# angelocatalani/neural-network-compression

Hardware: AMD Instinct MI355X
Metric: weights/sec through prune+k-means (K=256) (higher is better)
Workload: dtype f32

## Files before the change

### neural_network_compression_amd/csrc/nnc_layer.hip

```cpp
#include <hip/hip_runtime.h>

#include <algorithm>
#include <cmath>
#include <cstdint>
#include <cstring>
#include <string>
#include <vector>

#include "nnc.h"

int nnc_set_error_(int code, const char *msg);
int nnc_publish_bytes_(const void *src_dev, void *dst_host_mapped, int nbytes, void *host_ticket, uint64_t ticket, void *stream);
int nnc_wait_ticket_(void *host_ticket, uint64_t ticket, void *stream);
int nnc_sort_pruned_bounded_flagged_(const float *x, int64_t n, int64_t n_neg, int64_t n_zero, float vmin, float vmax, float thr,
                                     float *sorted_out, void *ws, size_t ws_bytes, int32_t *flag_dev, void *stream);
extern "C" int nnc_host_linspace_f32(float start, float stop, int32_t num, float *out)
{
    if (num < 0 || (num > 0 && !out)) return nnc_set_error_(NNC_EINVAL, "nnc_host_linspace_f32: bad argument");
    if (num == 0) return NNC_OK;
    const int div = num - 1;
    const volatile float delta = stop - start;
    if (div > 0) {
        const volatile float step = delta / (float)div;
        for (int i = 0; i < num; i++) {
            volatile float y = (float)i;
            if (step == 0.0f) { y = y / (float)div; y = y * delta; }
            else y = y * step;
            y = y + start;
            out[i] = y;
        }
        out[num - 1] = stop;
    } else {
        volatile float y = 0.0f;
        y = y * delta;
        y = y + start;
        out[0] = y;
    }
    return NNC_OK;
}

static void linspace_f64(double start, double stop, int num, double *out)
{
    const int div = num - 1;
    const volatile double delta = stop - start;
    if (div > 0) {
        const volatile double step = delta / (double)div;
        for (int i = 0; i < num; i++) {
            volatile double y = (double)i;
            if (step == 0.0) { y = y / (double)div; y = y * delta; }
            else y = y * step;
            y = y + start;
            out[i] = y;
        }
        out[num - 1] = stop;
    } else if (num == 1) {
        volatile double y = 0.0;
        y = y * delta;
        out[0] = y + start;
    }
}

extern "C" int nnc_host_cdf(const float *steps32, const int64_t *counts31, float *xnew300, double *cdf300)
{
    if (!steps32 || !counts31 || !xnew300 || !cdf300) return nnc_set_error_(NNC_EINVAL, "nnc_host_cdf: null pointer");
    const float *x = steps32;
    int64_t tot = 0;
// ... 108 lines not shown
    L.total = o + 256;
    return L;
}

extern "C" size_t nnc_compress_layer_workspace_bytes(int64_t n, int32_t k)
{
    if (n < 1 || k < 1 || k > NNC_KMAX - 8) return 0;
    return layer_layout(n, k).total;
}

extern "C" size_t nnc_compress_layer_host_bytes(void) { return 24576; }

#define LCHK(call) do { int rc_ = (call); if (rc_) return rc_; } while (0)
#define LHIP(call) do { hipError_t e_ = (call); if (e_ != hipSuccess) return nnc_set_error_(NNC_EHIP, hipGetErrorString(e_)); } while (0)

extern "C" int nnc_compress_layer_f32(float *x, int64_t n, const nnc_layer_params *lp, uint8_t *mask_out, void *labels_out,
                                      float *values_out, void *ws_dev, size_t ws_bytes, void *host_pinned, size_t host_bytes,
                                      uint64_t *ticket_io, nnc_layer_result *res, void *stream)
{
    if (!x || n < 1 || !lp || !labels_out || !ws_dev || !host_pinned || !ticket_io || !res)
        return nnc_set_error_(NNC_EINVAL, "nnc_compress_layer_f32: null pointer or empty tensor");
    if (lp->bits < 1 || lp->bits > 10 || (lp->mode != NNC_INIT_LINEAR && lp->mode != NNC_INIT_DENSITY))
        return nnc_set_error_(NNC_EINVAL, "nnc_compress_layer_f32: bits in 1..10, mode linear or density");
    if (lp->prune && !mask_out) return nnc_set_error_(NNC_EINVAL, "nnc_compress_layer_f32: pruning needs mask_out");
    const int32_t k = (1 << lp->bits) + (lp->mode == NNC_INIT_DENSITY ? 1 : 0);
    if (n < (int64_t)(1 << lp->bits) + 1) return nnc_set_error_(NNC_EINVAL, "nnc_compress_layer_f32: not enough weights for this many centroids");
    if (host_bytes < nnc_compress_layer_host_bytes() || (reinterpret_cast<uintptr_t>(host_pinned) & 7) != 0)
        return nnc_set_error_(NNC_EINVAL, "nnc_compress_layer_f32: host block too small or unaligned");
    const LayerLayout L = layer_layout(n, k);
    if (ws_bytes < L.total) return nnc_set_error_(NNC_ENOSPACE, "nnc_compress_layer_f32: workspace too small");
    hipStream_t s = reinterpret_cast<hipStream_t>(stream);
    unsigned char *wb = reinterpret_cast<unsigned char *>((reinterpret_cast<uintptr_t>(ws_dev) + 255) & ~(uintptr_t)255);
    unsigned char *hb = reinterpret_cast<unsigned char *>(host_pinned);
    const float *h_f = reinterpret_cast<const float *>(hb + 512);
    const int64_t *h_signs = reinterpret_cast<const int64_t *>(hb + 512 + 32);
    const float *h_prune = reinterpret_cast<const float *>(hb + 512 + 48);
    const int64_t *h_nz = reinterpret_cast<const int64_t *>(hb + 512 + 56);
    int64_t *h_ranks = reinterpret_cast<int64_t *>(hb + 576);
    void *h_ticket = hb + 504;
    auto read_back = [&](const void *src, void *dst, int nbytes) -> int {
        const uint64_t t = ++(*ticket_io);
        int rc = nnc_publish_bytes_(src, dst, nbytes, h_ticket, t, stream);
        if (rc) return rc;
        return nnc_wait_ticket_(h_ticket, t, stream);
    };
    std::memset(res, 0, sizeof(*res));
    res->k = k;
    res->label_bytes = k <= 256 ? 1 : 2;

    float *out6 = reinterpret_cast<float *>(wb + L.stats_out);
    int64_t *signs = reinterpret_cast<int64_t *>(wb + L.stats_out + 32);
    float *pstats = reinterpret_cast<float *>(wb + L.stats_out + 48);
    int64_t *nzeroed = reinterpret_cast<int64_t *>(wb + L.stats_out + 56);
    if (lp->prune)
        LCHK(nnc_prune_stats_f32(x, n, lp->q, lp->std_smooth ? 1 : 0, mask_out, pstats, nzeroed, out6 + 2, signs, wb + L.prune_ws, L.prune_ws_bytes, stream));
    else
        LCHK(nnc_minmax_signs_f32(x, n, out6 + 2, signs, wb + L.stats_ws, L.stats_ws_bytes, stream));
    const bool short_tensor = n <= NNC_REF_NMAX && k <= NNC_REF_KMAX;
    if ((short_tensor && lp->mode != NNC_INIT_LINEAR) || (!short_tensor && n < 512)) {
        if (lp->prune) {
            LCHK(read_back(out6, hb + 512, 64));
            res->sigma = h_prune[0]; res->threshold = h_prune[1]; res->n_zeroed = h_nz[0];
        }
        res->status = NNC_LAYER_HOST;
        return NNC_OK;
    }
    float space[NNC_KMAX];
    unsigned char *back = wb + L.back;
    int64_t *counts_d = reinterpret_cast<int64_t *>(back);
    float *centers_d = reinterpret_cast<float *>(back + (size_t)k * 8);
    int64_t *h_counts = reinterpret_cast<int64_t *>(hb + 1024);
    float *h_centers = reinterpret_cast<float *>(hb + 1024 + (size_t)k * 8);
    float *h_steps = reinterpret_cast<float *>(hb + 896), *h_space = reinterpret_cast<float *>(hb + 16384);

    if (short_tensor) {
        LCHK(read_back(out6, hb + 512, 64));
        LCHK(nnc_host_linspace_f32(h_f[2], h_f[3], k, space));
        std::memcpy(h_space, space, (size_t)k * 4);
        void *result_d = wb + L.small_out;
        LCHK(nnc_kmeans_fit_reference_f32(x, (int32_t)n, h_space, k, 300, 1e-4f, reinterpret_cast<uint8_t *>(labels_out), lp->want_values ? values_out : nullptr,
                                          centers_d, counts_d, result_d, stream));
        const int back_bytes = (int)al((size_t)k * 12) + 32;
        LCHK(read_back(back, hb + 1024, back_bytes));
        const int32_t *h_res = reinterpret_cast<const int32_t *>(hb + 1024 + al((size_t)k * 12));
        {
            const float *h_resf = reinterpret_cast<const float *>(h_res);
            if (!std::isfinite(h_resf[6]) || !std::isfinite(h_resf[7])) {
                if (lp->prune) { res->sigma = h_prune[0]; res->threshold = h_prune[1]; res->n_zeroed = h_nz[0]; }
                res->status = NNC_LAYER_HOST;
                return NNC_OK;
            }
        }
        res->n_iter = h_res[0]; res->stop = h_res[1]; res->n_relocations = h_res[2]; res->reloc_ties = h_res[3]; res->reloc_multi = h_res[4];
        res->arith = NNC_ARITH_REFERENCE;
    } else {
        const int64_t nch = (n + 8191) / 8192;
        float *c1 = reinterpret_cast<float *>(wb + L.stats_ws), *c2 = c1 + nch;
        SideStream *side = nullptr;
        LCHK(side_stream(&side));
        LHIP(hipEventRecord(side->fork, s));
        const uint64_t t_mm = ++(*ticket_io);
        LCHK(nnc_publish_bytes_(out6 + 2, hb + 512 + 8, 56, h_ticket, t_mm, stream));
        LHIP(hipStreamWaitEvent(side->stream, side->fork, 0));
        struct SideJoin {
            SideStream *side; hipStream_t s; bool joined = false;
            ~SideJoin() { if (!joined) { (void)hipEventRecord(side->join, side->stream); (void)hipStreamWaitEvent(s, side->join, 0); (void)hipStreamSynchronize(s); } }
        } side_join{side, s};
        LCHK(nnc_chunk_sums_f32(x, n, 0, nullptr, c1, side->stream));
        LCHK(nnc_fold_f32(c1, nch, n, NNC_FOLD_MEAN, nullptr, out6, side->stream));
        LCHK(nnc_chunk_sums_f32(x, n, 1, out6, c2, side->stream));
        LCHK(nnc_fold_f32(c2, nch, n, NNC_FOLD_MEAN, nullptr, out6 + 1, side->stream));
        void *h_ticket_side = hb + 864;
        const float *h_mv = reinterpret_cast<const float *>(hb + 872);
        const uint64_t t_mv = ++(*ticket_io);
        LCHK(nnc_publish_bytes_(out6, hb + 872, 8, h_ticket_side, t_mv, side->stream));
        LCHK(nnc_wait_ticket_(h_ticket, t_mm, stream));
        const float xmin = h_f[2], xmax = h_f[3], min_nz = h_f[4], max_nz = h_f[5];
        const int64_t n_neg = h_signs[0], n_zero = h_signs[1];
        float *xs = reinterpret_cast<float *>(wb + L.sorted);
        int32_t *oob_d = reinterpret_cast<int32_t *>(wb + L.stats_out + 336);
        const int32_t *h_oob = reinterpret_cast<const int32_t *>(hb + 512 + 336);
        bool bounded = false;
        if (4 * n_zero >= n && lp->prune && nnc_sort_pruned_bounded_bits(xmin, xmax, h_prune[1], n_neg, n - n_neg - n_zero) > 0) {
            LCHK(nnc_sort_pruned_bounded_flagged_(x, n, n_neg, n_zero, xmin, xmax, h_prune[1], xs, wb + L.sort_ws, L.sort_ws_bytes, oob_d, stream));
            bounded = true;
        } else if (4 * n_zero >= n) LCHK(nnc_sort_pruned_f32(x, n, n_neg, n_zero, xs, wb + L.sort_ws, L.sort_ws_bytes, stream));
        else LCHK(nnc_sort_f32(x, n, xs, wb + L.sort_ws, L.sort_ws_bytes, stream));
        LHIP(hipEventRecord(side->sorted, s));
        const bool with_prefix = (reinterpret_cast<uintptr_t>(xs) & 15) == 0;
        int64_t *ranks_d = reinterpret_cast<int64_t *>(wb + L.stats_out + 64);
        h_ranks = reinterpret_cast<int64_t *>(hb + 512 + 64);
        float steps[32];
        if (lp->mode == NNC_INIT_DENSITY) {
            if (!std::isfinite(min_nz)) {
                if (lp->prune) { res->sigma = h_prune[0]; res->threshold = h_prune[1]; res->n_zeroed = h_nz[0]; }
                res->status = NNC_LAYER_HOST;
                return NNC_OK;
            }
            LCHK(nnc_host_linspace_f32(min_nz, max_nz, 32, steps));
            std::memcpy(h_steps, steps, 128);
            LCHK(nnc_rank_sorted_f32(xs, n, h_steps, 32, ranks_d, stream));
        }
        const uint64_t t_rk = ++(*ticket_io);
        LCHK(nnc_publish_bytes_(out6 + 2, hb + 512 + 8, 56 + 33 * 8 + 16, h_ticket, t_rk, stream));
        LCHK(nnc_wait_ticket_(h_ticket_side, t_mv, side->stream));
        const float mean = h_mv[0], var = h_mv[1];
        if (!std::isfinite(mean) || !std::isfinite(var) || !std::isfinite(xmin) || !std::isfinite(xmax)) {
            LCHK(nnc_wait_ticket_(h_ticket, t_rk, stream));
            if (lp->prune) { res->sigma = h_prune[0]; res->threshold = h_prune[1]; res->n_zeroed = h_nz[0]; }
            res->status = NNC_LAYER_HOST;
            return NNC_OK;
        }
        nnc_kmeans_params p;
        std::memset(&p, 0, sizeof(p));
        const volatile float tol = var * 1e-4f;
// ... 61 lines not shown
```

### neural_network_compression_amd/csrc/nnc_reduce.hip

```cpp
#include "nnc_common.hpp"

#define LEAF_PAD 136
#define STEP_ELEMS 1024

template <bool SQDEV>
__device__ __forceinline__ float4 xform4(float4 v, float mean)
{
    if (SQDEV) {
        float a = v.x - mean, b = v.y - mean, c = v.z - mean, d = v.w - mean;
        v.x = a * a; v.y = b * b; v.z = c * c; v.w = d * d;
    }
    return v;
}

template <bool SQDEV>
__device__ __forceinline__ float xform1(float v, float mean)
{
    if (SQDEV) { float a = v - mean; return a * a; }
    return v;
}

struct PwFrame { int start, len, stage; float left; };

template <bool SQDEV, bool VEC>
__global__ __launch_bounds__(256) void k_chunk_sums(const float *__restrict__ x, int64_t nfull,
                                                    const float *__restrict__ mean_dev,
                                                    float *__restrict__ out, int tail)
{
    __shared__ __align__(16) float lds[4][8 * LEAF_PAD];
    __shared__ float nodes[8];
    const int wave = threadIdx.x >> 6, lane = threadIdx.x & 63;
    float *my = lds[wave];
    const float mean = SQDEV ? *mean_dev : 0.0f;
    const int64_t gmain = (int64_t)gridDim.x - (tail > 0 ? 1 : 0);
    if (tail > 0 && blockIdx.x == gridDim.x - 1) {
        __shared__ PwHeap heap;
        const float *xt = x + nfull * NNC_CHUNK;
        const float r = block_pairwise_sum([&](int i) { return xform1<SQDEV>(xt[i], mean); }, tail, &heap);
        if (threadIdx.x == 0) out[nfull] = r;
        return;
    }
    for (int64_t chunk = (int64_t)blockIdx.x; chunk < nfull; chunk += gmain) {
        const float *base = x + chunk * NNC_CHUNK + (int64_t)wave * 2 * STEP_ELEMS;
        float4 cur[2][4];
#pragma unroll
        for (int st = 0; st < 2; st++) {
#pragma unroll
            for (int r = 0; r < 4; r++) {
                if (VEC) cur[st][r] = reinterpret_cast<const float4 *>(base + st * STEP_ELEMS)[lane + 64 * r];
                else {
                    const float *p = base + st * STEP_ELEMS + 4 * (lane + 64 * r);
                    cur[st][r] = make_float4(p[0], p[1], p[2], p[3]);
                }
            }
        }
#pragma unroll
        for (int st = 0; st < 2; st++) {
#pragma unroll
            for (int r = 0; r < 4; r++) {
                int e = 4 * (lane + 64 * r);
                int b = e >> 7, pos = e & 127;
                *reinterpret_cast<float4 *>(&my[b * LEAF_PAD + pos]) = xform4<SQDEV>(cur[st][r], mean);
            }
            wave_lds_fence();
            const float *lp = &my[(lane >> 3) * LEAF_PAD + (lane & 7)];
            float acc = lp[0];
#pragma unroll
            for (int t = 1; t < 16; t++) acc = acc + lp[8 * t];
            wave_lds_fence();
            acc = acc + __shfl_xor(acc, 1);
            acc = acc + __shfl_xor(acc, 2);
            acc = acc + __shfl_xor(acc, 4);
            acc = acc + __shfl_xor(acc, 8);
            acc = acc + __shfl_xor(acc, 16);
            acc = acc + __shfl_xor(acc, 32);
            if (lane == 0) nodes[2 * wave + st] = acc;
        }
        __syncthreads();
        if (threadIdx.x == 0) out[chunk] = ((nodes[0] + nodes[1]) + (nodes[2] + nodes[3])) + ((nodes[4] + nodes[5]) + (nodes[6] + nodes[7]));
        __syncthreads();
    }
}

extern "C" int nnc_chunk_sums_f32(const float *x, int64_t n, int sqdev, const float *mean_dev,
                                  float *chunk_out, void *stream)
{
    if (n < 0 || (n > 0 && (!x || !chunk_out))) return fail(NNC_EINVAL, "nnc_chunk_sums_f32: null pointer");
    if (sqdev && !mean_dev) return fail(NNC_EINVAL, "nnc_chunk_sums_f32: sqdev needs mean_dev");
    if (n == 0) return NNC_OK;
    const int64_t nfull = n / NNC_CHUNK;
    const int tail = (int)(n % NNC_CHUNK);
    const bool vec = (reinterpret_cast<uintptr_t>(x) & 15) == 0;
    {
        int64_t blocks = nfull;
        int64_t cap = (int64_t)cu_count() * 16;
        int grid = (int)std::min<int64_t>(blocks, cap) + (tail > 0 ? 1 : 0);
        if (sqdev) {
            if (vec) NNC_LAUNCH_PROF(NNC_PROF_CHUNK_SUMS, (k_chunk_sums<true, true>), dim3(grid), dim3(256), 0, S(stream), x, nfull, mean_dev, chunk_out, tail);
            else NNC_LAUNCH_PROF(NNC_PROF_CHUNK_SUMS, (k_chunk_sums<true, false>), dim3(grid), dim3(256), 0, S(stream), x, nfull, mean_dev, chunk_out, tail);
        } else {
            if (vec) NNC_LAUNCH_PROF(NNC_PROF_CHUNK_SUMS, (k_chunk_sums<false, true>), dim3(grid), dim3(256), 0, S(stream), x, nfull, mean_dev, chunk_out, tail);
            else NNC_LAUNCH_PROF(NNC_PROF_CHUNK_SUMS, (k_chunk_sums<false, false>), dim3(grid), dim3(256), 0, S(stream), x, nfull, mean_dev, chunk_out, tail);
        }
        LAUNCHCHK("k_chunk_sums");
    }
    return NNC_OK;
}

#define FOLD_TILE 8192
__global__ __launch_bounds__(1024) void k_fold(const float *__restrict__ chunks, int64_t nchunks, int64_t count,
                                               int op, const float *__restrict__ scale_dev,
                                               float *__restrict__ out, float scale_val = 0.0f, int has_scale_val = 0,
                                               unsigned long long *__restrict__ zero64 = nullptr)
{
    if (zero64 && threadIdx.x == 0) *zero64 = 0ull;
    __shared__ __align__(16) float buf[FOLD_TILE];
    float acc = 0.0f;
    for (int64_t base = 0; base < nchunks; base += FOLD_TILE) {
        int len = (int)((nchunks - base) < FOLD_TILE ? (nchunks - base) : FOLD_TILE);
        for (int i = threadIdx.x; i < len; i += 1024) buf[i] = chunks[base + i];
        __syncthreads();
        if (threadIdx.x == 0) {
            const float4 *b4 = reinterpret_cast<const float4 *>(buf);
            const int nq = len >> 2;
            int qd = 0;
            for (; qd + 8 <= nq; qd += 8) {
                float4 v[8];
#pragma unroll
                for (int u = 0; u < 8; u++) v[u] = b4[qd + u];
#pragma unroll
                for (int u = 0; u < 8; u++) { acc = acc + v[u].x; acc = acc + v[u].y; acc = acc + v[u].z; acc = acc + v[u].w; }
            }
            for (; qd < nq; qd++) { const float4 v = b4[qd]; acc = acc + v.x; acc = acc + v.y; acc = acc + v.z; acc = acc + v.w; }
            for (int i = nq << 2; i < len; i++) acc = acc + buf[i];
        }
        __syncthreads();
    }
    if (threadIdx.x == 0) {
        float r = acc;
        if (op == NNC_FOLD_MEAN || op == NNC_FOLD_STD) r = (float)((double)acc / (double)count);
        if (op == NNC_FOLD_STD) r = (float)sqrt((double)r);
        out[0] = r;
        if (scale_dev) out[1] = r * (*scale_dev);
        else if (has_scale_val) out[1] = r * scale_val;
    }
}

extern "C" int nnc_fold_f32(const float *chunks, int64_t nchunks, int64_t count, int op, const float *scale_dev,
                            float *out_dev, void *stream)
{
    if (!out_dev || nchunks < 0 || (nchunks > 0 && !chunks)) return fail(NNC_EINVAL, "nnc_fold_f32: bad argument");
    if ((op == NNC_FOLD_MEAN || op == NNC_FOLD_STD) && count <= 0) return fail(NNC_EINVAL, "nnc_fold_f32: count <= 0");
    hipLaunchKernelGGL(k_fold, dim3(1), dim3(1024), 0, S(stream), chunks, nchunks, count, op, scale_dev, out_dev, 0.0f, 0, (unsigned long long *)nullptr);
    LAUNCHCHK("k_fold");
    return NNC_OK;
}

template <bool VEC>
__global__ __launch_bounds__(256) void k_threshold(float *__restrict__ x, int64_t n,
                                                   const float *__restrict__ thr_dev,
                                                   uint8_t *__restrict__ mask,
                                                   unsigned long long *__restrict__ nzeroed)
{
    const float thr = *thr_dev;
    unsigned cnt = 0;
    const int64_t tid = (int64_t)blockIdx.x * blockDim.x + threadIdx.x;
    const int64_t nthreads = (int64_t)gridDim.x * blockDim.x;
    int64_t done = 0;
    if (VEC) {
        const int64_t nvec = n >> 2;
        float4 *x4 = reinterpret_cast<float4 *>(x);
        uchar4 *m4 = reinterpret_cast<uchar4 *>(mask);
        for (int64_t v = tid; v < nvec; v += nthreads) {
            float4 a = x4[v];
            uchar4 m;
            m.x = fabsf(a.x) < thr; m.y = fabsf(a.y) < thr; m.z = fabsf(a.z) < thr; m.w = fabsf(a.w) < thr;
            cnt += m.x + m.y + m.z + m.w;
            a.x = m.x ? 0.0f : a.x; a.y = m.y ? 0.0f : a.y; a.z = m.z ? 0.0f : a.z; a.w = m.w ? 0.0f : a.w;
            x4[v] = a;
            m4[v] = m;
        }
        done = nvec << 2;
    }
    for (int64_t i = done + tid; i < n; i += nthreads) {
        float a = x[i];
        uint8_t m = fabsf(a) < thr;
        cnt += m;
        if (m) x[i] = 0.0f;
        mask[i] = m;
    }
// ... 97 lines not shown
    LAUNCHCHK("k_apply_mask");
    return NNC_OK;
}

struct MinMaxPartial { float mn, mx; unsigned long long cnt; unsigned long long neg, zer; float mn_nz, mx_nz; };

template <bool VEC>
__global__ __launch_bounds__(256) void k_minmax(const float *__restrict__ x, int64_t n, int skip_zeros,
                                                MinMaxPartial *__restrict__ part)
{
    float mn = INFINITY, mx = -INFINITY, mn_nz = INFINITY, mx_nz = -INFINITY;
    unsigned long long cnt = 0;
    unsigned neg = 0, zer = 0;
    const int64_t tid = (int64_t)blockIdx.x * blockDim.x + threadIdx.x;
    const int64_t nthreads = (int64_t)gridDim.x * blockDim.x;
    int64_t done = 0;
#define MM1(v) do { float v_ = (v); neg += (v_ < 0.0f); const bool z_ = (v_ == 0.0f); zer += z_; if (!z_) { mn_nz = fminf(mn_nz, v_); mx_nz = fmaxf(mx_nz, v_); } \
        bool use_ = !(skip_zeros && z_); if (use_) { mn = fminf(mn, v_); mx = fmaxf(mx, v_); cnt++; } } while (0)
    if (VEC) {
        const int64_t nvec = n >> 2;
        const float4 *x4 = reinterpret_cast<const float4 *>(x);
        for (int64_t v = tid; v < nvec; v += nthreads) {
            float4 a = x4[v];
            MM1(a.x); MM1(a.y); MM1(a.z); MM1(a.w);
        }
        done = nvec << 2;
    }
    for (int64_t i = done + tid; i < n; i += nthreads) MM1(x[i]);
#undef MM1
    unsigned long long negl = neg, zerl = zer;
    for (int off = 32; off > 0; off >>= 1) {
        mn = fminf(mn, __shfl_down(mn, off));
        mx = fmaxf(mx, __shfl_down(mx, off));
        mn_nz = fminf(mn_nz, __shfl_down(mn_nz, off));
        mx_nz = fmaxf(mx_nz, __shfl_down(mx_nz, off));
        cnt += __shfl_down(cnt, off);
        negl += __shfl_down(negl, off);
        zerl += __shfl_down(zerl, off);
    }
    __shared__ MinMaxPartial sh[4];
    if ((threadIdx.x & 63) == 0) { MinMaxPartial q; q.mn = mn; q.mx = mx; q.cnt = cnt; q.neg = negl; q.zer = zerl; q.mn_nz = mn_nz; q.mx_nz = mx_nz; sh[threadIdx.x >> 6] = q; }
    __syncthreads();
    if (threadIdx.x == 0) {
        MinMaxPartial p = sh[0];
        for (int w = 1; w < 4; w++) {
            p.mn = fminf(p.mn, sh[w].mn); p.mx = fmaxf(p.mx, sh[w].mx); p.cnt += sh[w].cnt; p.neg += sh[w].neg; p.zer += sh[w].zer;
            p.mn_nz = fminf(p.mn_nz, sh[w].mn_nz); p.mx_nz = fmaxf(p.mx_nz, sh[w].mx_nz);
        }
        part[blockIdx.x] = p;
    }
}

__global__ __launch_bounds__(256) void k_minmax_final(const MinMaxPartial *__restrict__ part, int nparts,
                                                      float *__restrict__ out, long long *__restrict__ count,
                                                      long long *__restrict__ signs)
{
    float mn = INFINITY, mx = -INFINITY, mn_nz = INFINITY, mx_nz = -INFINITY;
    unsigned long long cnt = 0, neg = 0, zer = 0;
    for (int i = threadIdx.x; i < nparts; i += 256) {
        mn = fminf(mn, part[i].mn); mx = fmaxf(mx, part[i].mx); cnt += part[i].cnt; neg += part[i].neg; zer += part[i].zer;
        mn_nz = fminf(mn_nz, part[i].mn_nz); mx_nz = fmaxf(mx_nz, part[i].mx_nz);
    }
    for (int off = 32; off > 0; off >>= 1) {
        mn = fminf(mn, __shfl_down(mn, off));
        mx = fmaxf(mx, __shfl_down(mx, off));
        mn_nz = fminf(mn_nz, __shfl_down(mn_nz, off));
        mx_nz = fmaxf(mx_nz, __shfl_down(mx_nz, off));
        cnt += __shfl_down(cnt, off);
        neg += __shfl_down(neg, off);
        zer += __shfl_down(zer, off);
    }
    __shared__ MinMaxPartial sh[4];
    if ((threadIdx.x & 63) == 0) { MinMaxPartial q; q.mn = mn; q.mx = mx; q.cnt = cnt; q.neg = neg; q.zer = zer; q.mn_nz = mn_nz; q.mx_nz = mx_nz; sh[threadIdx.x >> 6] = q; }
    __syncthreads();
    if (threadIdx.x == 0) {
        MinMaxPartial p = sh[0];
        for (int w = 1; w < 4; w++) {
            p.mn = fminf(p.mn, sh[w].mn); p.mx = fmaxf(p.mx, sh[w].mx); p.cnt += sh[w].cnt; p.neg += sh[w].neg; p.zer += sh[w].zer;
            p.mn_nz = fminf(p.mn_nz, sh[w].mn_nz); p.mx_nz = fmaxf(p.mx_nz, sh[w].mx_nz);
        }
        out[0] = p.mn; out[1] = p.mx;
        if (count) *count = (long long)p.cnt;
        if (signs) { signs[0] = (long long)p.neg; signs[1] = (long long)p.zer; out[2] = p.mn_nz; out[3] = p.mx_nz; }
    }
}

static int minmax_grid(int64_t n) { return stream_grid((n + 3) / 4, 256, 8); }

extern "C" size_t nnc_minmax_workspace_bytes(int64_t n)
{
    (void)n;
    return (size_t)(cu_count() * 8 + 8) * sizeof(MinMaxPartial);
}

static int minmax_impl(const float *x, int64_t n, int skip_zeros, float *out_dev, int64_t *count_dev, int64_t *signs_dev,
                       void *ws, size_t ws_bytes, void *stream)
{
    if (n <= 0 || !x || !out_dev || !ws) return fail(NNC_EINVAL, "nnc_minmax_f32: bad argument (n must be > 0)");
    if (ws_bytes < nnc_minmax_workspace_bytes(n)) return fail(NNC_ENOSPACE, "nnc_minmax_f32: workspace too small");
    int grid = minmax_grid(n);
    MinMaxPartial *part = reinterpret_cast<MinMaxPartial *>(ws);
    const bool vec = (reinterpret_cast<uintptr_t>(x) & 15) == 0;
    if (vec) NNC_LAUNCH_PROF(NNC_PROF_MINMAX, (k_minmax<true>), dim3(grid), dim3(256), 0, S(stream), x, n, skip_zeros, part);
    else NNC_LAUNCH_PROF(NNC_PROF_MINMAX, (k_minmax<false>), dim3(grid), dim3(256), 0, S(stream), x, n, skip_zeros, part);
    LAUNCHCHK("k_minmax");
    hipLaunchKernelGGL(k_minmax_final, dim3(1), dim3(256), 0, S(stream), part, grid, out_dev, reinterpret_cast<long long *>(count_dev),
                       reinterpret_cast<long long *>(signs_dev));
    LAUNCHCHK("k_minmax_final");
    return NNC_OK;
}

extern "C" int nnc_minmax_f32(const float *x, int64_t n, int skip_zeros, float *out_dev, int64_t *count_dev,
                              void *ws, size_t ws_bytes, void *stream)
{
    return minmax_impl(x, n, skip_zeros, out_dev, count_dev, nullptr, ws, ws_bytes, stream);
}

extern "C" int nnc_minmax_signs_f32(const float *x, int64_t n, float *out_dev, int64_t *signs_dev, void *ws, size_t ws_bytes,
                                    void *stream)
{
    if (!signs_dev) return fail(NNC_EINVAL, "nnc_minmax_signs_f32: null signs_dev");
    return minmax_impl(x, n, 0, out_dev, nullptr, signs_dev, ws, ws_bytes, stream);
}

template <bool VEC>
__global__ __launch_bounds__(256) void k_threshold_stats(float *__restrict__ x, int64_t n, const float *__restrict__ thr_dev,
                                                         uint8_t *__restrict__ mask, unsigned long long *__restrict__ nzeroed,
                                                         MinMaxPartial *__restrict__ part)
{
    const float thr = *thr_dev;
    unsigned cnt = 0, neg = 0, zer = 0;
    float mn = INFINITY, mx = -INFINITY, mn_nz = INFINITY, mx_nz = -INFINITY;
    const int64_t tid = (int64_t)blockIdx.x * blockDim.x + threadIdx.x;
    const int64_t nthreads = (int64_t)gridDim.x * blockDim.x;
    int64_t done = 0;
#define TS1(v) do { const float v_ = (v); neg += (v_ < 0.0f); const bool z_ = (v_ == 0.0f); zer += z_; \
        if (!z_) { mn_nz = fminf(mn_nz, v_); mx_nz = fmaxf(mx_nz, v_); } mn = fminf(mn, v_); mx = fmaxf(mx, v_); } while (0)
    if (VEC) {
        const int64_t nvec = n >> 2;
        float4 *x4 = reinterpret_cast<float4 *>(x);
        uchar4 *m4 = reinterpret_cast<uchar4 *>(mask);
        for (int64_t v = tid; v < nvec; v += nthreads) {
            float4 a = x4[v];
            uchar4 m;
            m.x = fabsf(a.x) < thr; m.y = fabsf(a.y) < thr; m.z = fabsf(a.z) < thr; m.w = fabsf(a.w) < thr;
            cnt += m.x + m.y + m.z + m.w;
            a.x = m.x ? 0.0f : a.x; a.y = m.y ? 0.0f : a.y; a.z = m.z ? 0.0f : a.z; a.w = m.w ? 0.0f : a.w;
            x4[v] = a;
            m4[v] = m;
            TS1(a.x); TS1(a.y); TS1(a.z); TS1(a.w);
        }
        done = nvec << 2;
    }
    for (int64_t i = done + tid; i < n; i += nthreads) {
        float a = x[i];
        const uint8_t m = fabsf(a) < thr;
        cnt += m;
        if (m) { a = 0.0f; x[i] = 0.0f; }
        mask[i] = m;
        TS1(a);
    }
#undef TS1
    unsigned long long negl = neg, zerl = zer, cntl = cnt;
    for (int off = 32; off > 0; off >>= 1) {
        mn = fminf(mn, __shfl_down(mn, off));
        mx = fmaxf(mx, __shfl_down(mx, off));
        mn_nz = fminf(mn_nz, __shfl_down(mn_nz, off));
        mx_nz = fmaxf(mx_nz, __shfl_down(mx_nz, off));
        negl += __shfl_down(negl, off);
        zerl += __shfl_down(zerl, off);
        cntl += __shfl_down(cntl, off);
    }
    __shared__ MinMaxPartial sh[4];
    __shared__ unsigned long long shc[4];
    if ((threadIdx.x & 63) == 0) {
        MinMaxPartial q; q.mn = mn; q.mx = mx; q.cnt = 0; q.neg = negl; q.zer = zerl; q.mn_nz = mn_nz; q.mx_nz = mx_nz;
        sh[threadIdx.x >> 6] = q; shc[threadIdx.x >> 6] = cntl;
    }
    __syncthreads();
    if (threadIdx.x == 0) {
        MinMaxPartial p = sh[0];
        unsigned long long tot = shc[0];
        for (int w = 1; w < 4; w++) {
            p.mn = fminf(p.mn, sh[w].mn); p.mx = fmaxf(p.mx, sh[w].mx); p.neg += sh[w].neg; p.zer += sh[w].zer;
            p.mn_nz = fminf(p.mn_nz, sh[w].mn_nz); p.mx_nz = fmaxf(p.mx_nz, sh[w].mx_nz);
            tot += shc[w];
        }
        part[blockIdx.x] = p;
        if (nzeroed && tot) atomicAdd(nzeroed, tot);
    }
}

extern "C" size_t nnc_prune_stats_workspace_bytes(int64_t n) { return ((nnc_prune_workspace_bytes(n) + 255) & ~(size_t)255) + nnc_minmax_workspace_bytes(n); }

extern "C" int nnc_prune_stats_f32(float *x, int64_t n, float q, int std_smooth, uint8_t *mask, float *stats_dev, int64_t *nzeroed_dev,
                                   float *minmax4_dev, int64_t *signs_dev, void *ws, size_t ws_bytes, void *stream)
{
    if (n <= 0 || !x || !mask || !stats_dev || !minmax4_dev || !signs_dev || !ws) return fail(NNC_EINVAL, "nnc_prune_stats_f32: bad argument (n must be > 0)");
    if (ws_bytes < nnc_prune_stats_workspace_bytes(n)) return fail(NNC_ENOSPACE, "nnc_prune_stats_f32: workspace too small");
    if (std_smooth) {
        float *wsf = reinterpret_cast<float *>(ws);
        float *scal = wsf;
        float *chunks = wsf + 16;
        const int64_t nchunks = (n + NNC_CHUNK - 1) / NNC_CHUNK;
        int rc;
        if ((rc = nnc_chunk_sums_f32(x, n, 0, nullptr, chunks, stream))) return rc;
        if ((rc = nnc_fold_f32(chunks, nchunks, n, NNC_FOLD_MEAN, nullptr, scal, stream))) return rc;
        if ((rc = nnc_chunk_sums_f32(x, n, 1, scal, chunks, stream))) return rc;
        hipLaunchKernelGGL(k_fold, dim3(1), dim3(1024), 0, S(stream), chunks, nchunks, n, (int)NNC_FOLD_STD, (const float *)nullptr, stats_dev, q, 1,
                           reinterpret_cast<unsigned long long *>(nzeroed_dev));
        LAUNCHCHK("k_fold");
    } else {
        hipLaunchKernelGGL(k_set_thr, dim3(1), dim3(1), 0, S(stream), q, stats_dev);
        LAUNCHCHK("k_set_thr");
        if (nzeroed_dev) HIPCHK(hipMemsetAsync(nzeroed_dev, 0, sizeof(int64_t), S(stream)));
    }
    MinMaxPartial *part = reinterpret_cast<MinMaxPartial *>(reinterpret_cast<unsigned char *>(ws) + ((nnc_prune_workspace_bytes(n) + 255) & ~(size_t)255));
    const bool vec = ((reinterpret_cast<uintptr_t>(x) & 15) == 0) && ((reinterpret_cast<uintptr_t>(mask) & 3) == 0);
    const int grid = std::min(stream_grid((n + 3) / 4, 256, 4), cu_count() * 8);
    if (vec) NNC_LAUNCH_PROF(NNC_PROF_THRESHOLD, (k_threshold_stats<true>), dim3(grid), dim3(256), 0, S(stream), x, n, stats_dev + 1, mask, reinterpret_cast<unsigned long long *>(nzeroed_dev), part);
    else NNC_LAUNCH_PROF(NNC_PROF_THRESHOLD, (k_threshold_stats<false>), dim3(grid), dim3(256), 0, S(stream), x, n, stats_dev + 1, mask, reinterpret_cast<unsigned long long *>(nzeroed_dev), part);
    LAUNCHCHK("k_threshold_stats");
    hipLaunchKernelGGL(k_minmax_final, dim3(1), dim3(256), 0, S(stream), part, grid, minmax4_dev, (long long *)nullptr, reinterpret_cast<long long *>(signs_dev));
    LAUNCHCHK("k_minmax_final");
    return NNC_OK;
}

extern "C" size_t nnc_layer_stats_workspace_bytes(int64_t n)
{
    const size_t nch = (size_t)((n + NNC_CHUNK - 1) / NNC_CHUNK);
    return ((2 * nch * sizeof(float) + 255) & ~(size_t)255) + nnc_minmax_workspace_bytes(n);
}

extern "C" int nnc_layer_stats_f32(const float *x, int64_t n, float *out6_dev, int64_t *signs_dev, void *ws, size_t ws_bytes,
                                   void *stream)
{
    if (n <= 0 || !x || !out6_dev || !signs_dev || !ws) return fail(NNC_EINVAL, "nnc_layer_stats_f32: bad argument (n must be > 0)");
    if (ws_bytes < nnc_layer_stats_workspace_bytes(n)) return fail(NNC_ENOSPACE, "nnc_layer_stats_f32: workspace too small");
    const int64_t nch = (n + NNC_CHUNK - 1) / NNC_CHUNK;
    float *c1 = reinterpret_cast<float *>(ws), *c2 = c1 + nch;
    unsigned char *mm_ws = reinterpret_cast<unsigned char *>(ws) + ((2 * (size_t)nch * sizeof(float) + 255) & ~(size_t)255);
    int rc;
    if ((rc = nnc_chunk_sums_f32(x, n, 0, nullptr, c1, stream))) return rc;
    if ((rc = nnc_fold_f32(c1, nch, n, NNC_FOLD_MEAN, nullptr, out6_dev, stream))) return rc;
    if ((rc = nnc_chunk_sums_f32(x, n, 1, out6_dev, c2, stream))) return rc;
    if ((rc = nnc_fold_f32(c2, nch, n, NNC_FOLD_MEAN, nullptr, out6_dev + 1, stream))) return rc;
    return minmax_impl(x, n, 0, out6_dev + 2, nullptr, signs_dev, mm_ws, nnc_minmax_workspace_bytes(n), stream);
}

template <bool VEC>
__global__ __launch_bounds__(256) void k_hist31(const float *__restrict__ x, int64_t n, int skip_zeros,
                                                const float *__restrict__ steps,
                                                unsigned long long *__restrict__ counts)
{
    __shared__ unsigned h[32][32];
    __shared__ float st[32];
    for (int i = threadIdx.x; i < 32 * 32; i += 256) (&h[0][0])[i] = 0;
    if (threadIdx.x < 32) st[threadIdx.x] = steps[threadIdx.x];
    __syncthreads();
    float s[32];
#pragma unroll
    for (int i = 0; i < 32; i++) s[i] = st[i];
    const int rep = threadIdx.x & 31;
    const int64_t tid = (int64_t)blockIdx.x * blockDim.x + threadIdx.x;
    const int64_t nthreads = (int64_t)gridDim.x * blockDim.x;
#define H1(v) do { float v_ = (v); if (!(skip_zeros && v_ == 0.0f)) { int c_ = 0; _Pragma("unroll") for (int i = 0; i < 32; i++) c_ += (v_ >= s[i]); if (c_ >= 1 && c_ <= 31) atomicAdd(&h[c_ - 1][rep], 1u); } } while (0)
    int64_t done = 0;
    if (VEC) {
        const int64_t nvec = n >> 2;
        const float4 *x4 = reinterpret_cast<const float4 *>(x);
        for (int64_t v = tid; v < nvec; v += nthreads) {
            float4 a = x4[v];
            H1(a.x); H1(a.y); H1(a.z); H1(a.w);
        }
        done = nvec << 2;
    }
    for (int64_t i = done + tid; i < n; i += nthreads) H1(x[i]);
#undef H1
    __syncthreads();
    if (threadIdx.x < 31) {
        unsigned long long t = 0;
        for (int r = 0; r < 32; r++) t += h[threadIdx.x][r];
        if (t) atomicAdd(&counts[threadIdx.x], t);
    }
}

extern "C" int nnc_hist31_f32(const float *x, int64_t n, int skip_zeros, const float *steps32_dev,
                              int64_t *counts_dev, void *stream)
{
    if (n < 0 || !steps32_dev || !counts_dev || (n > 0 && !x)) return fail(NNC_EINVAL, "nnc_hist31_f32: bad argument");
    if (n == 0) return NNC_OK;
    int grid = stream_grid((n + 3) / 4, 256, 2);
    const bool vec = (reinterpret_cast<uintptr_t>(x) & 15) == 0;
    if (vec) hipLaunchKernelGGL((k_hist31<true>), dim3(grid), dim3(256), 0, S(stream), x, n, skip_zeros, steps32_dev, reinterpret_cast<unsigned long long *>(counts_dev));
    else hipLaunchKernelGGL((k_hist31<false>), dim3(grid), dim3(256), 0, S(stream), x, n, skip_zeros, steps32_dev, reinterpret_cast<unsigned long long *>(counts_dev));
    LAUNCHCHK("k_hist31");
    return NNC_OK;
}
// ... 57 lines not shown
```

Before: 10.43 billion.

## Fold mean/std reductions into consumer kernels and publish prune stats from device

The separate single-block fold kernels are folded into the next consumer. The squared-deviation chunk-sum kernel and the threshold-stats kernel now each compute the mean or sigma redundantly per workgroup, while their first loads are already in flight. The serial one-thread fold is replaced by a 64-lane staged fold that keeps the same summation order. The host read-back of min/max/signs is written directly by k_minmax_final to mapped host memory with a ticket, removing a separate publish launch. The cost is that every block re-reads the chunk-sum array, and the threshold kernel launches with 1024 threads and a larger grid.

```diff
diff --git a/neural_network_compression_amd/csrc/nnc_layer.hip b/neural_network_compression_amd/csrc/nnc_layer.hip
--- a/neural_network_compression_amd/csrc/nnc_layer.hip
+++ b/neural_network_compression_amd/csrc/nnc_layer.hip
@@ -12,6 +12,10 @@
 int nnc_set_error_(int code, const char *msg);
 int nnc_publish_bytes_(const void *src_dev, void *dst_host_mapped, int nbytes, void *host_ticket, uint64_t ticket, void *stream);
 int nnc_wait_ticket_(void *host_ticket, uint64_t ticket, void *stream);
+int nnc_chunk_sums_folded_(const float *x, int64_t n, const float *sums, float *mean_out, int64_t *zero64, float *chunk_out, void *stream);
+int nnc_prune_stats_publish_(float *x, int64_t n, float q, int std_smooth, uint8_t *mask, float *stats_dev, int64_t *nzeroed_dev,
+                             float *minmax4_dev, int64_t *signs_dev, void *ws, size_t ws_bytes, const void *pub_src, void *pub_dst_host,
+                             int pub_bytes, void *host_ticket, uint64_t ticket, void *stream);
 int nnc_sort_pruned_bounded_flagged_(const float *x, int64_t n, int64_t n_neg, int64_t n_zero, float vmin, float vmax, float thr,
                                      float *sorted_out, void *ws, size_t ws_bytes, int32_t *flag_dev, void *stream);
 extern "C" int nnc_host_linspace_f32(float start, float stop, int32_t num, float *out)
@@ -226,12 +230,18 @@
     int64_t *signs = reinterpret_cast<int64_t *>(wb + L.stats_out + 32);
     float *pstats = reinterpret_cast<float *>(wb + L.stats_out + 48);
     int64_t *nzeroed = reinterpret_cast<int64_t *>(wb + L.stats_out + 56);
-    if (lp->prune)
+    const bool short_tensor = n <= NNC_REF_NMAX && k <= NNC_REF_KMAX;
+    const bool not_taken = (short_tensor && lp->mode != NNC_INIT_LINEAR) || (!short_tensor && n < 512);
+    uint64_t t_mm = 0;
+    if (lp->prune && !short_tensor && !not_taken) {
+        t_mm = ++(*ticket_io);
+        LCHK(nnc_prune_stats_publish_(x, n, lp->q, lp->std_smooth ? 1 : 0, mask_out, pstats, nzeroed, out6 + 2, signs, wb + L.prune_ws, L.prune_ws_bytes,
+                                      out6 + 2, hb + 512 + 8, 56, h_ticket, t_mm, stream));
+    } else if (lp->prune)
         LCHK(nnc_prune_stats_f32(x, n, lp->q, lp->std_smooth ? 1 : 0, mask_out, pstats, nzeroed, out6 + 2, signs, wb + L.prune_ws, L.prune_ws_bytes, stream));
     else
         LCHK(nnc_minmax_signs_f32(x, n, out6 + 2, signs, wb + L.stats_ws, L.stats_ws_bytes, stream));
-    const bool short_tensor = n <= NNC_REF_NMAX && k <= NNC_REF_KMAX;
-    if ((short_tensor && lp->mode != NNC_INIT_LINEAR) || (!short_tensor && n < 512)) {
+    if (not_taken) {
         if (lp->prune) {
             LCHK(read_back(out6, hb + 512, 64));
             res->sigma = h_prune[0]; res->threshold = h_prune[1]; res->n_zeroed = h_nz[0];
@@ -273,8 +283,10 @@
         SideStream *side = nullptr;
         LCHK(side_stream(&side));
         LHIP(hipEventRecord(side->fork, s));
-        const uint64_t t_mm = ++(*ticket_io);
-        LCHK(nnc_publish_bytes_(out6 + 2, hb + 512 + 8, 56, h_ticket, t_mm, stream));
+        if (!lp->prune) {
+            t_mm = ++(*ticket_io);
+            LCHK(nnc_publish_bytes_(out6 + 2, hb + 512 + 8, 56, h_ticket, t_mm, stream));
+        }
         LHIP(hipStreamWaitEvent(side->stream, side->fork, 0));
         struct SideJoin {
             SideStream *side; hipStream_t s; bool joined = false;
diff --git a/neural_network_compression_amd/csrc/nnc_reduce.hip b/neural_network_compression_amd/csrc/nnc_reduce.hip
--- a/neural_network_compression_amd/csrc/nnc_reduce.hip
+++ b/neural_network_compression_amd/csrc/nnc_reduce.hip
@@ -22,27 +22,67 @@
 
 struct PwFrame { int start, len, stage; float left; };
 
-template <bool SQDEV, bool VEC>
-__global__ __launch_bounds__(256) void k_chunk_sums(const float *__restrict__ x, int64_t nfull,
-                                                    const float *__restrict__ mean_dev,
-                                                    float *__restrict__ out, int tail)
+#define FOLD_PER 48
+#define FOLD_STAGE (64 * FOLD_PER)
+__device__ __forceinline__ float fold_tile(const float *buf, int len, float acc)
+{
+    const int lane = threadIdx.x & 63;
+    float v[FOLD_PER];
+    const float4 *b4 = reinterpret_cast<const float4 *>(buf + lane * FOLD_PER);
+#pragma unroll
+    for (int u = 0; u < FOLD_PER / 4; u++) { const float4 t = b4[u]; v[4 * u] = t.x; v[4 * u + 1] = t.y; v[4 * u + 2] = t.z; v[4 * u + 3] = t.w; }
+    const int rounds = (len + FOLD_PER - 1) / FOLD_PER;
+#pragma unroll 1
+    for (int r = 0; r < rounds; r++) {
+        float a = acc;
+#pragma unroll
+        for (int j = 0; j < FOLD_PER; j++) a = a + v[j];
+        acc = __int_as_float(__builtin_amdgcn_readlane(__float_as_int(a), r));
+    }
+    return acc;
+}
+
+template <int THREADS>
+__device__ __forceinline__ float wg_fold_sums(const float *__restrict__ chunks, int64_t nchunks, float *buf, float *bcast)
+{
+    static_assert(FOLD_STAGE % THREADS == 0, "a tile is a whole number of loads a thread");
+    float acc = 0.0f;
+    for (int64_t base = 0; base < nchunks; base += FOLD_STAGE) {
+        const int len = (int)((nchunks - base) < FOLD_STAGE ? (nchunks - base) : FOLD_STAGE);
+        float stage[FOLD_STAGE / THREADS];
+#pragma unroll
+        for (int u = 0; u < FOLD_STAGE / THREADS; u++) {
+            const int i = (int)threadIdx.x + u * THREADS;
+            stage[u] = i < len ? chunks[base + i] : 0.0f;
+        }
+#pragma unroll
+        for (int u = 0; u < FOLD_STAGE / THREADS; u++) buf[(int)threadIdx.x + u * THREADS] = stage[u];
+        __syncthreads();
+        if (threadIdx.x < 64) acc = fold_tile(buf, len, acc);
+        __syncthreads();
+    }
+    if (threadIdx.x == 0) *bcast = acc;
+    __syncthreads();
+    return *bcast;
+}
+
+struct FoldIn { const float *sums; int64_t nsums, count; float *mean_out; unsigned long long *zero64; };
+
+template <bool SQDEV, bool VEC, bool FOLD>
+__device__ __forceinline__ void chunk_sums_body(const float *__restrict__ x, int64_t nfull, const float *__restrict__ mean_dev,
+                                                float *__restrict__ out, int tail, const FoldIn f)
 {
     __shared__ __align__(16) float lds[4][8 * LEAF_PAD];
     __shared__ float nodes[8];
+    __shared__ float folded;
+    static_assert(FOLD_STAGE <= 4 * 8 * LEAF_PAD, "the fold's stage is the transposition buffer");
     const int wave = threadIdx.x >> 6, lane = threadIdx.x & 63;
     float *my = lds[wave];
-    const float mean = SQDEV ? *mean_dev : 0.0f;
     const int64_t gmain = (int64_t)gridDim.x - (tail > 0 ? 1 : 0);
-    if (tail > 0 && blockIdx.x == gridDim.x - 1) {
-        __shared__ PwHeap heap;
-        const float *xt = x + nfull * NNC_CHUNK;
-        const float r = block_pairwise_sum([&](int i) { return xform1<SQDEV>(xt[i], mean); }, tail, &heap);
-        if (threadIdx.x == 0) out[nfull] = r;
-        return;
-    }
-    for (int64_t chunk = (int64_t)blockIdx.x; chunk < nfull; chunk += gmain) {
+    const bool ragged = tail > 0 && blockIdx.x == gridDim.x - 1;
+    float4 cur[2][4];
+    auto load_chunk = [&](int64_t chunk) {
         const float *base = x + chunk * NNC_CHUNK + (int64_t)wave * 2 * STEP_ELEMS;
-        float4 cur[2][4];
 #pragma unroll
         for (int st = 0; st < 2; st++) {
 #pragma unroll
@@ -54,6 +94,26 @@
                 }
             }
         }
+    };
+    float mean = 0.0f;
+    if (FOLD) {
+        if (!ragged) load_chunk((int64_t)blockIdx.x);
+        const float acc = wg_fold_sums<256>(f.sums, f.nsums, &lds[0][0], &folded);
+        mean = (float)((double)acc / (double)f.count);
+        if (blockIdx.x == 0 && threadIdx.x == 0) {
+            *f.mean_out = mean;
+            if (f.zero64) *f.zero64 = 0ull;
+        }
+    } else if (SQDEV) mean = *mean_dev;
+    if (ragged) {
+        __shared__ PwHeap heap;
+        const float *xt = x + nfull * NNC_CHUNK;
+        const float r = block_pairwise_sum([&](int i) { return xform1<SQDEV>(xt[i], mean); }, tail, &heap);
+        if (threadIdx.x == 0) out[nfull] = r;
+        return;
+    }
+    for (int64_t chunk = (int64_t)blockIdx.x; chunk < nfull; chunk += gmain) {
+        if (!FOLD || chunk != (int64_t)blockIdx.x) load_chunk(chunk);
 #pragma unroll
         for (int st = 0; st < 2; st++) {
 #pragma unroll
@@ -80,6 +140,21 @@
         if (threadIdx.x == 0) out[chunk] = ((nodes[0] + nodes[1]) + (nodes[2] + nodes[3])) + ((nodes[4] + nodes[5]) + (nodes[6] + nodes[7]));
         __syncthreads();
     }
+}
+
+template <bool SQDEV, bool VEC>
+__global__ __launch_bounds__(256) void k_chunk_sums(const float *__restrict__ x, int64_t nfull,
+                                                    const float *__restrict__ mean_dev,
+                                                    float *__restrict__ out, int tail)
+{
+    chunk_sums_body<SQDEV, VEC, false>(x, nfull, mean_dev, out, tail, FoldIn{});
+}
+
+template <bool VEC>
+__global__ __launch_bounds__(256) void k_chunk_sums_folded(const float *__restrict__ x, int64_t nfull, float *__restrict__ out, int tail,
+                                                           const FoldIn f)
+{
+    chunk_sums_body<true, VEC, true>(x, nfull, nullptr, out, tail, f);
 }
 
 extern "C" int nnc_chunk_sums_f32(const float *x, int64_t n, int sqdev, const float *mean_dev,
@@ -107,35 +182,32 @@
     return NNC_OK;
 }
 
-#define FOLD_TILE 8192
+#define NNC_FOLDED_PER_CU 4
+int nnc_chunk_sums_folded_(const float *x, int64_t n, const float *sums, float *mean_out, int64_t *zero64, float *chunk_out, void *stream)
+{
+    if (n <= 0 || !x || !sums || !mean_out || !chunk_out) return fail(NNC_EINVAL, "chunk sums behind a mean pass: bad argument");
+    const int64_t nfull = n / NNC_CHUNK;
+    const int tail = (int)(n % NNC_CHUNK);
+    const bool vec = (reinterpret_cast<uintptr_t>(x) & 15) == 0;
+    const int64_t cap = (int64_t)cu_count() * NNC_FOLDED_PER_CU;
+    const int64_t rounds = (nfull + cap - 1) / cap;
+    const int grid = (int)(rounds > 0 ? (nfull + rounds - 1) / rounds : 0) + (tail > 0 ? 1 : 0);
+    const FoldIn f{sums, nfull + (tail > 0 ? 1 : 0), n, mean_out, reinterpret_cast<unsigned long long *>(zero64)};
+    if (vec) NNC_LAUNCH_PROF(NNC_PROF_CHUNK_SUMS, (k_chunk_sums_folded<true>), dim3(grid), dim3(256), 0, S(stream), x, nfull, chunk_out, tail, f);
+    else NNC_LAUNCH_PROF(NNC_PROF_CHUNK_SUMS, (k_chunk_sums_folded<false>), dim3(grid), dim3(256), 0, S(stream), x, nfull, chunk_out, tail, f);
+    LAUNCHCHK("k_chunk_sums_folded");
+    return NNC_OK;
+}
+
 __global__ __launch_bounds__(1024) void k_fold(const float *__restrict__ chunks, int64_t nchunks, int64_t count,
                                                int op, const float *__restrict__ scale_dev,
                                                float *__restrict__ out, float scale_val = 0.0f, int has_scale_val = 0,
                                                unsigned long long *__restrict__ zero64 = nullptr)
 {
     if (zero64 && threadIdx.x == 0) *zero64 = 0ull;
-    __shared__ __align__(16) float buf[FOLD_TILE];
-    float acc = 0.0f;
-    for (int64_t base = 0; base < nchunks; base += FOLD_TILE) {
-        int len = (int)((nchunks - base) < FOLD_TILE ? (nchunks - base) : FOLD_TILE);
-        for (int i = threadIdx.x; i < len; i += 1024) buf[i] = chunks[base + i];
-        __syncthreads();
-        if (threadIdx.x == 0) {
-            const float4 *b4 = reinterpret_cast<const float4 *>(buf);
-            const int nq = len >> 2;
-            int qd = 0;
-            for (; qd + 8 <= nq; qd += 8) {
-                float4 v[8];
-#pragma unroll
-                for (int u = 0; u < 8; u++) v[u] = b4[qd + u];
-#pragma unroll
-                for (int u = 0; u < 8; u++) { acc = acc + v[u].x; acc = acc + v[u].y; acc = acc + v[u].z; acc = acc + v[u].w; }
-            }
-            for (; qd < nq; qd++) { const float4 v = b4[qd]; acc = acc + v.x; acc = acc + v.y; acc = acc + v.z; acc = acc + v.w; }
-            for (int i = nq << 2; i < len; i++) acc = acc + buf[i];
-        }
-        __syncthreads();
-    }
+    __shared__ __align__(16) float buf[FOLD_STAGE];
+    __shared__ float folded;
+    const float acc = wg_fold_sums<1024>(chunks, nchunks, buf, &folded);
     if (threadIdx.x == 0) {
         float r = acc;
         if (op == NNC_FOLD_MEAN || op == NNC_FOLD_STD) r = (float)((double)acc / (double)count);
@@ -339,8 +411,9 @@
 }
 
 __global__ __launch_bounds__(256) void k_minmax_final(const MinMaxPartial *__restrict__ part, int nparts,
-                                                      float *__restrict__ out, long long *__restrict__ count,
-                                                      long long *__restrict__ signs)
+                                                      float *out, long long *count, long long *signs,
+                                                      const unsigned long long *pub_src = nullptr, unsigned long long *pub_dst_host = nullptr,
+                                                      int pub_words = 0, unsigned long long *host_ticket = nullptr, unsigned long long ticket = 0ull)
 {
     float mn = INFINITY, mx = -INFINITY, mn_nz = INFINITY, mx_nz = -INFINITY;
     unsigned long long cnt = 0, neg = 0, zer = 0;
@@ -369,6 +442,12 @@
         out[0] = p.mn; out[1] = p.mx;
         if (count) *count = (long long)p.cnt;
         if (signs) { signs[0] = (long long)p.neg; signs[1] = (long long)p.zer; out[2] = p.mn_nz; out[3] = p.mx_nz; }
+        if (pub_dst_host) {
+            __threadfence();
+            for (int i = 0; i < pub_words; i++) pub_dst_host[i] = *reinterpret_cast<const volatile unsigned long long *>(pub_src + i);
+            __threadfence_system();
+            *reinterpret_cast<volatile unsigned long long *>(host_ticket) = ticket;
+        }
     }
 }
 
@@ -392,7 +471,8 @@
     else NNC_LAUNCH_PROF(NNC_PROF_MINMAX, (k_minmax<false>), dim3(grid), dim3(256), 0, S(stream), x, n, skip_zeros, part);
     LAUNCHCHK("k_minmax");
     hipLaunchKernelGGL(k_minmax_final, dim3(1), dim3(256), 0, S(stream), part, grid, out_dev, reinterpret_cast<long long *>(count_dev),
-                       reinterpret_cast<long long *>(signs_dev));
+                       reinterpret_cast<long long *>(signs_dev), (const unsigned long long *)nullptr, (unsigned long long *)nullptr, 0,
+                       (unsigned long long *)nullptr, 0ull);
     LAUNCHCHK("k_minmax_final");
     return NNC_OK;
 }
@@ -410,16 +490,29 @@
     return minmax_impl(x, n, 0, out_dev, nullptr, signs_dev, ws, ws_bytes, stream);
 }
 
-template <bool VEC>
-__global__ __launch_bounds__(256) void k_threshold_stats(float *__restrict__ x, int64_t n, const float *__restrict__ thr_dev,
+struct SigmaIn { const float *sums; int64_t nsums, count; float q; float *stats_out; };
+
+template <bool VEC, bool FOLD, int THREADS>
+__global__ __launch_bounds__(THREADS) void k_threshold_stats(float *__restrict__ x, int64_t n, const float *__restrict__ thr_dev,
                                                          uint8_t *__restrict__ mask, unsigned long long *__restrict__ nzeroed,
-                                                         MinMaxPartial *__restrict__ part)
-{
-    const float thr = *thr_dev;
+                                                         MinMaxPartial *__restrict__ part, const SigmaIn f)
+{
+    const int64_t tid = (int64_t)blockIdx.x * blockDim.x + threadIdx.x;
+    const int64_t nthreads = (int64_t)gridDim.x * blockDim.x;
+    float thr;
+    float4 first = make_float4(0.0f, 0.0f, 0.0f, 0.0f);
+    if (FOLD) {
+        __shared__ __align__(16) float stage[FOLD_STAGE];
+        __shared__ float folded;
+        if (VEC && tid < (n >> 2)) first = reinterpret_cast<const float4 *>(x)[tid];
+        const float acc = wg_fold_sums<THREADS>(f.sums, f.nsums, stage, &folded);
+        float r = (float)((double)acc / (double)f.count);
+        r = (float)sqrt((double)r);
+        thr = r * f.q;
+        if (blockIdx.x == 0 && threadIdx.x == 0) { f.stats_out[0] = r; f.stats_out[1] = thr; }
+    } else thr = *thr_dev;
     unsigned cnt = 0, neg = 0, zer = 0;
     float mn = INFINITY, mx = -INFINITY, mn_nz = INFINITY, mx_nz = -INFINITY;
-    const int64_t tid = (int64_t)blockIdx.x * blockDim.x + threadIdx.x;
-    const int64_t nthreads = (int64_t)gridDim.x * blockDim.x;
     int64_t done = 0;
 #define TS1(v) do { const float v_ = (v); neg += (v_ < 0.0f); const bool z_ = (v_ == 0.0f); zer += z_; \
         if (!z_) { mn_nz = fminf(mn_nz, v_); mx_nz = fmaxf(mx_nz, v_); } mn = fminf(mn, v_); mx = fmaxf(mx, v_); } while (0)
@@ -428,7 +521,7 @@
         float4 *x4 = reinterpret_cast<float4 *>(x);
         uchar4 *m4 = reinterpret_cast<uchar4 *>(mask);
         for (int64_t v = tid; v < nvec; v += nthreads) {
-            float4 a = x4[v];
+            float4 a = (FOLD && v == tid) ? first : x4[v];
             uchar4 m;
             m.x = fabsf(a.x) < thr; m.y = fabsf(a.y) < thr; m.z = fabsf(a.z) < thr; m.w = fabsf(a.w) < thr;
             cnt += m.x + m.y + m.z + m.w;
@@ -458,8 +551,8 @@
         zerl += __shfl_down(zerl, off);
         cntl += __shfl_down(cntl, off);
     }
-    __shared__ MinMaxPartial sh[4];
-    __shared__ unsigned long long shc[4];
+    __shared__ MinMaxPartial sh[THREADS / 64];
+    __shared__ unsigned long long shc[THREADS / 64];
     if ((threadIdx.x & 63) == 0) {
         MinMaxPartial q; q.mn = mn; q.mx = mx; q.cnt = 0; q.neg = negl; q.zer = zerl; q.mn_nz = mn_nz; q.mx_nz = mx_nz;
         sh[threadIdx.x >> 6] = q; shc[threadIdx.x >> 6] = cntl;
@@ -468,7 +561,7 @@
     if (threadIdx.x == 0) {
         MinMaxPartial p = sh[0];
         unsigned long long tot = shc[0];
-        for (int w = 1; w < 4; w++) {
+        for (int w = 1; w < THREADS / 64; w++) {
             p.mn = fminf(p.mn, sh[w].mn); p.mx = fmaxf(p.mx, sh[w].mx); p.neg += sh[w].neg; p.zer += sh[w].zer;
             p.mn_nz = fminf(p.mn_nz, sh[w].mn_nz); p.mx_nz = fmaxf(p.mx_nz, sh[w].mx_nz);
             tot += shc[w];
@@ -478,39 +571,61 @@
     }
 }
 
-extern "C" size_t nnc_prune_stats_workspace_bytes(int64_t n) { return ((nnc_prune_workspace_bytes(n) + 255) & ~(size_t)255) + nnc_minmax_workspace_bytes(n); }
-
-extern "C" int nnc_prune_stats_f32(float *x, int64_t n, float q, int std_smooth, uint8_t *mask, float *stats_dev, int64_t *nzeroed_dev,
-                                   float *minmax4_dev, int64_t *signs_dev, void *ws, size_t ws_bytes, void *stream)
+static size_t prune_stats_sums_bytes(int64_t n)
+{
+    const int64_t nchunks = (n + NNC_CHUNK - 1) / NNC_CHUNK;
+    return (((size_t)(2 * nchunks + 64) * sizeof(float)) + 255) & ~(size_t)255;
+}
+
+extern "C" size_t nnc_prune_stats_workspace_bytes(int64_t n) { return prune_stats_sums_bytes(n) + nnc_minmax_workspace_bytes(n); }
+
+int nnc_prune_stats_publish_(float *x, int64_t n, float q, int std_smooth, uint8_t *mask, float *stats_dev, int64_t *nzeroed_dev,
+                             float *minmax4_dev, int64_t *signs_dev, void *ws, size_t ws_bytes, const void *pub_src, void *pub_dst_host,
+                             int pub_bytes, void *host_ticket, uint64_t ticket, void *stream)
 {
     if (n <= 0 || !x || !mask || !stats_dev || !minmax4_dev || !signs_dev || !ws) return fail(NNC_EINVAL, "nnc_prune_stats_f32: bad argument (n must be > 0)");
     if (ws_bytes < nnc_prune_stats_workspace_bytes(n)) return fail(NNC_ENOSPACE, "nnc_prune_stats_f32: workspace too small");
+    if (pub_dst_host && (!pub_src || !host_ticket || pub_bytes < 0 || (pub_bytes & 7) || ((reinterpret_cast<uintptr_t>(pub_src) | reinterpret_cast<uintptr_t>(pub_dst_host)) & 7)))
+        return fail(NNC_EINVAL, "nnc_prune_stats_f32: bad host read");
+    SigmaIn sg{nullptr, 0, 0, 0.0f, nullptr};
     if (std_smooth) {
         float *wsf = reinterpret_cast<float *>(ws);
         float *scal = wsf;
-        float *chunks = wsf + 16;
         const int64_t nchunks = (n + NNC_CHUNK - 1) / NNC_CHUNK;
+        float *c1 = wsf + 16, *c2 = c1 + nchunks;
         int rc;
-        if ((rc = nnc_chunk_sums_f32(x, n, 0, nullptr, chunks, stream))) return rc;
-        if ((rc = nnc_fold_f32(chunks, nchunks, n, NNC_FOLD_MEAN, nullptr, scal, stream))) return rc;
-        if ((rc = nnc_chunk_sums_f32(x, n, 1, scal, chunks, stream))) return rc;
-        hipLaunchKernelGGL(k_fold, dim3(1), dim3(1024), 0, S(stream), chunks, nchunks, n, (int)NNC_FOLD_STD, (const float *)nullptr, stats_dev, q, 1,
-                           reinterpret_cast<unsigned long long *>(nzeroed_dev));
-        LAUNCHCHK("k_fold");
+        if ((rc = nnc_chunk_sums_f32(x, n, 0, nullptr, c1, stream))) return rc;
+        if ((rc = nnc_chunk_sums_folded_(x, n, c1, scal, nzeroed_dev, c2, stream))) return rc;
+        sg = SigmaIn{c2, nchunks, n, q, stats_dev};
     } else {
         hipLaunchKernelGGL(k_set_thr, dim3(1), dim3(1), 0, S(stream), q, stats_dev);
         LAUNCHCHK("k_set_thr");
         if (nzeroed_dev) HIPCHK(hipMemsetAsync(nzeroed_dev, 0, sizeof(int64_t), S(stream)));
     }
-    MinMaxPartial *part = reinterpret_cast<MinMaxPartial *>(reinterpret_cast<unsigned char *>(ws) + ((nnc_prune_workspace_bytes(n) + 255) & ~(size_t)255));
+    MinMaxPartial *part = reinterpret_cast<MinMaxPartial *>(reinterpret_cast<unsigned char *>(ws) + prune_stats_sums_bytes(n));
     const bool vec = ((reinterpret_cast<uintptr_t>(x) & 15) == 0) && ((reinterpret_cast<uintptr_t>(mask) & 3) == 0);
-    const int grid = std::min(stream_grid((n + 3) / 4, 256, 4), cu_count() * 8);
-    if (vec) NNC_LAUNCH_PROF(NNC_PROF_THRESHOLD, (k_threshold_stats<true>), dim3(grid), dim3(256), 0, S(stream), x, n, stats_dev + 1, mask, reinterpret_cast<unsigned long long *>(nzeroed_dev), part);
-    else NNC_LAUNCH_PROF(NNC_PROF_THRESHOLD, (k_threshold_stats<false>), dim3(grid), dim3(256), 0, S(stream), x, n, stats_dev + 1, mask, reinterpret_cast<unsigned long long *>(nzeroed_dev), part);
+    const int grid = std_smooth ? stream_grid((n + 3) / 4, 1024, 1) : std::min(stream_grid((n + 3) / 4, 256, 4), cu_count() * 8);
+    unsigned long long *nz = reinterpret_cast<unsigned long long *>(nzeroed_dev);
+    if (std_smooth) {
+        if (vec) NNC_LAUNCH_PROF(NNC_PROF_THRESHOLD, (k_threshold_stats<true, true, 1024>), dim3(grid), dim3(1024), 0, S(stream), x, n, (const float *)nullptr, mask, nz, part, sg);
+        else NNC_LAUNCH_PROF(NNC_PROF_THRESHOLD, (k_threshold_stats<false, true, 1024>), dim3(grid), dim3(1024), 0, S(stream), x, n, (const float *)nullptr, mask, nz, part, sg);
+    } else {
+        if (vec) NNC_LAUNCH_PROF(NNC_PROF_THRESHOLD, (k_threshold_stats<true, false, 256>), dim3(grid), dim3(256), 0, S(stream), x, n, stats_dev + 1, mask, nz, part, sg);
+        else NNC_LAUNCH_PROF(NNC_PROF_THRESHOLD, (k_threshold_stats<false, false, 256>), dim3(grid), dim3(256), 0, S(stream), x, n, stats_dev + 1, mask, nz, part, sg);
+    }
     LAUNCHCHK("k_threshold_stats");
-    hipLaunchKernelGGL(k_minmax_final, dim3(1), dim3(256), 0, S(stream), part, grid, minmax4_dev, (long long *)nullptr, reinterpret_cast<long long *>(signs_dev));
+    hipLaunchKernelGGL(k_minmax_final, dim3(1), dim3(256), 0, S(stream), part, grid, minmax4_dev, (long long *)nullptr, reinterpret_cast<long long *>(signs_dev),
+                       reinterpret_cast<const unsigned long long *>(pub_src), reinterpret_cast<unsigned long long *>(pub_dst_host), pub_bytes / 8,
+                       reinterpret_cast<unsigned long long *>(host_ticket), (unsigned long long)ticket);
     LAUNCHCHK("k_minmax_final");
     return NNC_OK;
+}
+
+extern "C" int nnc_prune_stats_f32(float *x, int64_t n, float q, int std_smooth, uint8_t *mask, float *stats_dev, int64_t *nzeroed_dev,
+                                   float *minmax4_dev, int64_t *signs_dev, void *ws, size_t ws_bytes, void *stream)
+{
+    return nnc_prune_stats_publish_(x, n, q, std_smooth, mask, stats_dev, nzeroed_dev, minmax4_dev, signs_dev, ws, ws_bytes, nullptr, nullptr, 0, nullptr, 0,
+                                    stream);
 }
 
 extern "C" size_t nnc_layer_stats_workspace_bytes(int64_t n)
@@ -529,8 +644,7 @@
     unsigned char *mm_ws = reinterpret_cast<unsigned char *>(ws) + ((2 * (size_t)nch * sizeof(float) + 255) & ~(size_t)255);
     int rc;
     if ((rc = nnc_chunk_sums_f32(x, n, 0, nullptr, c1, stream))) return rc;
-    if ((rc = nnc_fold_f32(c1, nch, n, NNC_FOLD_MEAN, nullptr, out6_dev, stream))) return rc;
-    if ((rc = nnc_chunk_sums_f32(x, n, 1, out6_dev, c2, stream))) return rc;
+    if ((rc = nnc_chunk_sums_folded_(x, n, c1, out6_dev, nullptr, c2, stream))) return rc;
     if ((rc = nnc_fold_f32(c2, nch, n, NNC_FOLD_MEAN, nullptr, out6_dev + 1, stream))) return rc;
     return minmax_impl(x, n, 0, out6_dev + 2, nullptr, signs_dev, mm_ws, nnc_minmax_workspace_bytes(n), stream);
 }
```

Result: faster. 10.58 billion, median of 6 (+1.4%).
